# AIGeeksGroup/UniVid

Hardware: AMD Instinct MI355X
Metric: denoise_steps_per_sec (higher is better)
Workload: dtype bf16

## Files before the change

### include/univid_hip.h

```cpp
#ifndef UNIVID_HIP_H
#define UNIVID_HIP_H
#include <stdint.h>
#ifdef __cplusplus
extern "C" {
#endif

int uv_version(void);
const char* uv_build_id(void);
int uv_init(void);
const char* uv_last_error(void);
int uv_device_arch(char* buf, int len);
int uv_host_blocking_sync(int on);

#define UV_OPT_CONV_HALO 0
#define UV_OPT_GEMM_GM 1
#define UV_OPT_ATTN_CUT 2
int uv_set_option(int key, int value);
int uv_get_option(int key, int* value);
int uv_reset_options(void);

#define UV_EPI_BF16 0
#define UV_EPI_GELU_BF16 1
#define UV_EPI_F32_FROM_BF16 2
#define UV_EPI_RESID_F32 3
#define UV_EPI_GATE_RESID_F32 4
#define UV_EPI_BF16_T 5

int uv_gemm_bf16_nt(const void* A, long lda, const void* W, long ldw, const void* bias_bf16, int M, int N, int K,
                    int epilogue, void* out, long ldo, const float* gate, const int32_t* gate_tid, long gate_stride,
                    int tile_cfg, void* stream);

int uv_gemm_bf16_nt_ws(const void* A, long lda, const void* W, long ldw, const void* bias_bf16, int M, int N, int K,
                       int epilogue, void* out, long ldo, const float* gate, const int32_t* gate_tid, long gate_stride,
                       int tile_cfg, void* workspace, long workspace_bytes, void* stream);
long uv_gemm_splitk_ws_bytes(int M, int N, int K);

int uv_gemm_f16_nt(const void* A, long lda, const void* W, long ldw, const void* bias_f16, int M, int N, int K, int epilogue,
                   void* out, long ldo, const float* gate, const int32_t* gate_tid, long gate_stride, int tile_cfg, void* stream);

int uv_gemm_bf16_nt_ssq(const void* A, long lda, const void* W, long ldw, const void* bias_bf16, int M, int N, int K, void* out, long ldo,
                        float* ssq, long ld_ssq, int tile_cfg, void* stream);
int uv_rms_scale_from_ssq(const float* ssq, long ld_ssq, int M, int groups, int C, float eps, float* rs, void* stream);

int uv_gemm_f32_nt(const float* A, long lda, const float* W, long ldw, const float* bias, int M, int N, int K, float* out,
                   long ldo, const float* resid, long ldr, void* stream);

int uv_flash_attn_bf16(const void* q, long ldq, const void* k, long ldk, const void* vt, long ldvt, void* out, long ldo,
                       int batch, int Lq, int Lk, int H, int head_dim, float softmax_scale, void* stream);

int uv_flash_attn_bf16_qnorm(const void* q, long ldq, const void* k, long ldk, const void* vt, long ldvt, void* out, long ldo,
                             int batch, int Lq, int Lk, int H, int head_dim, float softmax_scale, const float* q_rs, const float* q_weight,
                             void* stream);

int uv_flash_attn_f16(const void* q, long ldq, const void* k, long ldk, const void* vt, long ldvt, void* out, long ldo,
                      int batch, int Lq, int Lk, int H, int head_dim, float softmax_scale, void* stream);

int uv_flash_attn_kernel_name(int Lk, int head_dim, long ldk, long ldvt, int f16, char* buf, int len);

int uv_transpose_16(const void* in, long ldi, void* out, long ldo, int L, int C, int Lpad, void* stream);
int uv_cast_f32_to16(const float* in, void* out, long n, int f16, void* stream);
int uv_cast_16_to_f32(const void* in, float* out, long n, int f16, void* stream);

int uv_t5_attention_bf16(const void* q, long ldq, const void* k, long ldk, const void* v, long ldv, void* out, long ldo, int n, int H,
                         const float* rel_bias, int span, void* stream);

int uv_layernorm_mod(const float* x, long ldx, void* out, long ldo, int L, int C, float eps, int mode, const float* tab,
                     long tab_stride, int shift_off, int scale_off, const int32_t* tid, const float* w, const float* b,
                     int round_ln, int out_bf16, void* stream);
// ... 67 lines not shown
```

### univid_amd/_lib.py

```python
import ctypes
import os

import torch

_HERE = os.path.dirname(os.path.abspath(__file__))
LIB_PATH = os.path.join(_HERE, "libunivid_hip.so")

_c = ctypes
_P, _L, _I, _F = _c.c_void_p, _c.c_long, _c.c_int, _c.c_float

SIGNATURES = {
    "uv_version": [],
    "uv_init": [],
    "uv_last_error": [],
    "uv_build_id": [],
    "uv_device_arch": [_c.c_char_p, _I],
    "uv_host_blocking_sync": [_I],
    "uv_set_option": [_I, _I],
    "uv_get_option": [_I, _c.POINTER(_I)],
    "uv_reset_options": [],
    "uv_gemm_bf16_nt": [_P, _L, _P, _L, _P, _I, _I, _I, _I, _P, _L, _P, _P, _L, _I, _P],
    "uv_gemm_bf16_nt_ws": [_P, _L, _P, _L, _P, _I, _I, _I, _I, _P, _L, _P, _P, _L, _I, _P, _L, _P],
    "uv_gemm_splitk_ws_bytes": [_I, _I, _I],
    "uv_gemm_f16_nt": [_P, _L, _P, _L, _P, _I, _I, _I, _I, _P, _L, _P, _P, _L, _I, _P],
    "uv_gemm_f32_nt": [_P, _L, _P, _L, _P, _I, _I, _I, _P, _L, _P, _L, _P],
    "uv_gemm_bf16_nt_ssq": [_P, _L, _P, _L, _P, _I, _I, _I, _P, _L, _P, _L, _I, _P],
    "uv_rms_scale_from_ssq": [_P, _L, _I, _I, _I, _F, _P, _P],
    "uv_flash_attn_bf16_qnorm": [_P, _L, _P, _L, _P, _L, _P, _L, _I, _I, _I, _I, _I, _F, _P, _P, _P],
    "uv_flash_attn_bf16": [_P, _L, _P, _L, _P, _L, _P, _L, _I, _I, _I, _I, _I, _F, _P],
    "uv_flash_attn_f16": [_P, _L, _P, _L, _P, _L, _P, _L, _I, _I, _I, _I, _I, _F, _P],
    "uv_flash_attn_kernel_name": [_I, _I, _L, _L, _I, _c.c_char_p, _I],
    "uv_transpose_16": [_P, _L, _P, _L, _I, _I, _I, _P],
    "uv_cast_f32_to16": [_P, _P, _L, _I, _P],
    "uv_cast_16_to_f32": [_P, _P, _L, _I, _P],
    "uv_layernorm_mod": [_P, _L, _P, _L, _I, _I, _F, _I, _P, _L, _I, _I, _P, _P, _P, _I, _I, _P],
    "uv_t5_attention_bf16": [_P, _L, _P, _L, _P, _L, _P, _L, _I, _I, _P, _I, _P],
    "uv_add_bf16": [_P, _P, _P, _L, _P],
    "uv_t5_gated_gelu_bf16": [_P, _P, _P, _L, _P],
    "uv_gelu_erf_bf16": [_P, _P, _L, _P],
    "uv_interp_linear_rows_bf16": [_P, _L, _P, _L, _I, _I, _I, _P],
    "uv_l2_normalize_rows_f32": [_P, _L, _P, _L, _I, _I, _F, _P],
    "uv_rmsnorm_rope": [_P, _L, _P, _L, _P, _I, _I, _I, _F, _P, _I, _I, _I, _I, _P],
    "uv_rmsnorm_rope_qk": [_P, _P, _P, _P, _P, _P, _L, _L, _I, _I, _I, _I, _F, _P, _I, _I, _I, _I, _P],
    "uv_patchify_bf16": [_P, _P, _L, _I, _I, _I, _I, _I, _I, _I, _I, _P],
    "uv_unpatchify_f32": [_P, _L, _P, _I, _I, _I, _I, _I, _I, _I, _P],
    "uv_sinusoid_f32": [_P, _P, _I, _I, _P],
    "uv_linear_rows_f32": [_P, _L, _P, _P, _P, _L, _I, _I, _I, _I, _P],
    "uv_add_rows_f32": [_P, _P, _P, _I, _L, _P],
    "uv_cast_f32_bf16": [_P, _P, _L, _P],
    "uv_add_bf16_resid": [_P, _L, _P, _L, _I, _I, _P],
    "uv_text_weight_rows_bf16": [_P, _L, _P, _L, _I, _I, _I, _F, _P],
    "uv_cfg_convert": [_P, _P, _P, _F, _F, _P, _P, _L, _P],
    "uv_unipc_corrector": [_P, _P, _P, _P, _P, _F, _F, _F, _F, _F, _F, _I, _L, _P],
    "uv_unipc_predictor": [_P, _P, _P, _P, _F, _F, _F, _F, _I, _L, _P],
    "uv_dpmpp_update": [_P, _P, _P, _P, _F, _F, _F, _I, _L, _P],
    "uv_conv3d_f32": [_P, _L, _I, _I, _I, _P, _P, _P, _L, _I, _I, _I, _I, _I, _I, _I, _I, _I, _I, _I, _I, _I, _I, _I, _I,
# ... 157 lines not shown
        raise UnividHipError(f"{name} failed ({rc}): {lib.uv_last_error().decode()}")
    if timed:
        e.record(stream)
        prof.setdefault(name, []).append((s, e, flops))



def _chk(t, dtype, name):
    if t.device.type != "cuda":
        raise UnividHipError(f"{name}: tensor must live on the GPU (got {t.device})")
    if t.dtype != dtype:
        raise UnividHipError(f"{name}: expected {dtype}, got {t.dtype}")
    if t.stride(-1) != 1:
        raise UnividHipError(f"{name}: innermost dimension must be contiguous")


def host_blocking_sync(on=True, device=None):
    dev = torch.device("cuda" if device is None else device)
    idx = torch.cuda.current_device() if dev.index is None else dev.index
    lib = load()
    with torch.cuda.device(idx):
        if lib.uv_host_blocking_sync(1 if on else 0) != 0:
            raise UnividHipError(lib.uv_last_error().decode())


def gemm_splitk_ws_bytes(M, N, K, device=None):
    dev = torch.device("cuda" if device is None else device)
    idx = torch.cuda.current_device() if dev.index is None else dev.index
    lib = init(idx)
    with torch.cuda.device(idx):
        return int(lib.uv_gemm_splitk_ws_bytes(int(M), int(N), int(K)))


def gemm_bf16(a, w, bias, out, epi, M=None, gate=None, gate_tid=None, tile_cfg=0, ws=None):
    f16 = a.dtype == torch.float16
    _chk(a, torch.float16 if f16 else torch.bfloat16, "gemm_bf16.a")
    _chk(w, a.dtype, "gemm_bf16.w")
    M = a.shape[0] if M is None else M
    N, K = w.shape
    if ws is not None and not f16:
        _chk(ws, torch.uint8, "gemm_bf16.ws")
        call("uv_gemm_bf16_nt_ws", ptr(a), a.stride(0), ptr(w), w.stride(0), ptr(bias), M, N, K, epi, ptr(out), out.stride(0),
             ptr(gate), ptr(gate_tid), 0 if gate is None else gate.stride(0), tile_cfg, ptr(ws), ws.numel(), stream_ptr(), flops=2 * M * N * K)
        return out
    call("uv_gemm_f16_nt" if f16 else "uv_gemm_bf16_nt", ptr(a), a.stride(0), ptr(w), w.stride(0), ptr(bias), M, N, K, epi, ptr(out), out.stride(0),
         ptr(gate), ptr(gate_tid), 0 if gate is None else gate.stride(0), tile_cfg, stream_ptr(), flops=2 * M * N * K)
    return out


def gemm_bf16_ssq(a, w, bias, out, ssq, M=None, tile_cfg=0):
    _chk(a, torch.bfloat16, "gemm_bf16_ssq.a")
    _chk(w, torch.bfloat16, "gemm_bf16_ssq.w")
    _chk(ssq, torch.float32, "gemm_bf16_ssq.ssq")
    M = a.shape[0] if M is None else M
    N, K = w.shape
    call("uv_gemm_bf16_nt_ssq", ptr(a), a.stride(0), ptr(w), w.stride(0), ptr(bias), M, N, K, ptr(out), out.stride(0), ptr(ssq), ssq.stride(0),
         tile_cfg, stream_ptr(), flops=2 * M * N * K)
    return out


def rms_scale_from_ssq(ssq, rs, M, C, eps):
    _chk(ssq, torch.float32, "rms_scale_from_ssq.ssq")
    _chk(rs, torch.float32, "rms_scale_from_ssq.rs")
    call("uv_rms_scale_from_ssq", ptr(ssq), ssq.stride(0), M, ssq.shape[1], C, float(eps), ptr(rs), stream_ptr())
    return rs

# ... 69 lines not shown
```

### univid_amd/csrc/gemm_bf16.hip

```cpp
#include "gemm_bf16_kernels.h"

int uv_gemm_diag_launch(const GemmArgs& a, int epilogue, int tile_cfg, hipStream_t s);

static int num_cus() { return uv_num_cus(); }

template <bool F16>
static int launch_by_cfg(const GemmArgs& a, int epilogue, int tile_cfg, hipStream_t s);

struct GemmWs {
    void* p = nullptr;
    long bytes = 0;
};

template <bool F16>
static bool strip_takes_splitk(const GemmArgs& at, int epilogue, const GemmWs& ws) {
    if (F16 || !ws.p) return false;
    if (epilogue != UV_EPI_BF16 && epilogue != UV_EPI_RESID_F32 && epilogue != UV_EPI_GATE_RESID_F32) return false;
    if (at.K < 8192 || at.K % 512 != 0 || at.N % 256 != 0) return false;
    const long tiles = (long)((at.M + 255) / 256) * (at.N / 256);
    return tiles * 4 <= num_cus() && ws.bytes >= splitk_ws_bytes(at.M, at.N, 4) && ((uintptr_t)ws.p & 255) == 0;
}

static long persistent_rows(int M, int N, bool* short_round) {
    const long tn = N / 256, tm_full = M / 256;
// ... 19 lines not shown
    if (a.gate_tid) at.gate_tid = a.gate_tid + m_main;
    if (epilogue == UV_EPI_BF16_T) at.out = (bf16_t*)a.out + m_main;
    else if (epilogue == UV_EPI_BF16 || epilogue == UV_EPI_GELU_BF16 || epilogue == UV_EPI_BF16_SSQ) at.out = (bf16_t*)a.out + m_main * a.ldo;
    else at.out = (float*)a.out + m_main * a.ldo;
    if (a.ssq) at.ssq = a.ssq + m_main * a.ld_ssq;
    const int rc = launch_by_cfg<F16>(am, epilogue, main_cfg, s);
    if (rc) return rc;
    if constexpr (!F16)
        if (strip_takes_splitk<F16>(at, epilogue, ws)) return launch_8ph_splitk<4, false>(at, epilogue, s, ws.p, ws.bytes);
    return launch_by_cfg<F16>(at, epilogue, 12, s);
}

template <bool F16>
static int gemm_entry(const void* A, long lda, const void* W, long ldw, const void* bias_bf16, int M, int N, int K, int epilogue,
                      void* out, long ldo, const float* gate, const int32_t* gate_tid, long gate_stride, int tile_cfg, void* stream,
                      float* ssq = nullptr, long ld_ssq = 0, const GemmWs& ws = GemmWs()) {
    UV_CHECK_ARG(A && W && out, "uv_gemm_bf16_nt: null pointer");
    UV_CHECK_ARG(M > 0 && N > 0 && K > 0, "uv_gemm_bf16_nt: bad shape M=%d N=%d K=%d", M, N, K);
    UV_CHECK_ARG(K % UV_BK == 0, "uv_gemm_bf16_nt: K=%d must be a multiple of %d", K, UV_BK);
    UV_CHECK_ARG(N % 16 == 0, "uv_gemm_bf16_nt: N=%d must be a multiple of 16", N);
    UV_CHECK_ARG(lda % 8 == 0 && ldw % 8 == 0, "uv_gemm_bf16_nt: lda/ldw must be multiples of 8 elements");
    UV_CHECK_ARG(((uintptr_t)A & 15) == 0 && ((uintptr_t)W & 15) == 0 && ((uintptr_t)out & 15) == 0,
                 "uv_gemm_bf16_nt: pointers must be 16-byte aligned");
    UV_CHECK_ARG(ldo % 4 == 0, "uv_gemm_bf16_nt: ldo must be a multiple of 4 elements");
    if (epilogue == UV_EPI_GATE_RESID_F32)
        UV_CHECK_ARG(gate && gate_stride % 4 == 0, "uv_gemm_bf16_nt: gate table required (stride %% 4 == 0)");
    GemmArgs a;
    a.A = (const bf16_t*)A; a.W = (const bf16_t*)W; a.bias = (const bf16_t*)bias_bf16;
    a.out = out; a.gate = gate; a.gate_tid = gate_tid;
    a.lda = lda; a.ldw = ldw; a.ldo = ldo; a.gate_stride = gate_stride;
    a.M = M; a.N = N; a.K = K; a.tiles_m = a.tiles_n = 0;
    a.ssq = ssq; a.ld_ssq = ld_ssq;
    a.ws_slab = nullptr; a.ws_cnt = nullptr; a.gm = 0;
    if (epilogue == UV_EPI_BF16_SSQ)
        UV_CHECK_ARG(ssq && N % 32 == 0 && ld_ssq >= N / 32 && ldo % 8 == 0, "uv_gemm_bf16_nt_ssq: needs N %% 32 == 0, ld_ssq >= N / 32, ldo %% 8 == 0 (N=%d ld_ssq=%ld ldo=%ld)", N, ld_ssq, ldo);
    a.zeros = uv_zero_page();
    UV_CHECK_ARG(a.zeros, "uv_gemm_bf16_nt: zero page missing (call uv_init)");
    hipStream_t s = (hipStream_t)stream;
    if (tile_cfg == 0 && M >= 2048 && N >= 1024 && N % 256 == 0 && K % 128 == 0 && K >= 384 &&
        (ldo % 8 == 0 || epilogue == UV_EPI_BF16_T || (epilogue >= UV_EPI_F32_FROM_BF16 && epilogue != UV_EPI_BF16_SSQ))) {
        const long tn = N / 256;
        bool short_round = false;
        const long m_main = persistent_rows(M, N, &short_round);
        if (m_main / 256 * tn < 2L * num_cus() || (epilogue == UV_EPI_BF16_T && ldo % 8 != 0)) {
            if (short_round) return launch_m_split<F16>(a, epilogue, 7, s);
            return launch_by_cfg<F16>(a, epilogue, 7, s);
        }
        return launch_m_split<F16>(a, epilogue, 17, s, m_main, ws);
    }
    if constexpr (!F16) {
        if (tile_cfg == 19) return launch_8ph_splitk<4, false>(a, epilogue, s, ws.p, ws.bytes);
        if (tile_cfg == 20) return launch_8ph_splitk<2, false>(a, epilogue, s, ws.p, ws.bytes);
        if (tile_cfg == 21) { a.gm = 1; return launch_8ph_splitk<4, false>(a, epilogue, s, ws.p, ws.bytes); }
    }
    if (tile_cfg == 8) return launch_m_split<F16>(a, epilogue, 7, s);
    if (tile_cfg == 9) return launch_m_split<F16>(a, epilogue, 5, s);
    if (tile_cfg == 18) return launch_m_split<F16>(a, epilogue, 17, s, (long)(M / 256) * 256 < M ? (long)(M / 256) * 256 : 0);
    return launch_by_cfg<F16>(a, epilogue, tile_cfg, s);
}

extern "C" int uv_gemm_bf16_nt(const void* A, long lda, const void* W, long ldw, const void* bias_bf16,
                               int M, int N, int K, int epilogue, void* out, long ldo,
                               const float* gate, const int32_t* gate_tid, long gate_stride,
                               int tile_cfg, void* stream) {
    return gemm_entry<false>(A, lda, W, ldw, bias_bf16, M, N, K, epilogue, out, ldo, gate, gate_tid, gate_stride, tile_cfg, stream);
}

extern "C" int uv_gemm_bf16_nt_ws(const void* A, long lda, const void* W, long ldw, const void* bias_bf16,
                                  int M, int N, int K, int epilogue, void* out, long ldo,
                                  const float* gate, const int32_t* gate_tid, long gate_stride,
                                  int tile_cfg, void* workspace, long workspace_bytes, void* stream) {
    UV_CHECK_ARG(workspace_bytes >= 0 && (workspace || workspace_bytes == 0), "uv_gemm_bf16_nt_ws: bad workspace");
    GemmWs ws;
    ws.p = workspace; ws.bytes = workspace_bytes;
    return gemm_entry<false>(A, lda, W, ldw, bias_bf16, M, N, K, epilogue, out, ldo, gate, gate_tid, gate_stride, tile_cfg, stream, nullptr, 0, ws);
}

extern "C" long uv_gemm_splitk_ws_bytes(int M, int N, int K) {
    if (M < 2048 || N < 1024 || N % 256 != 0 || K < 8192 || K % 512 != 0) return 0;
    const long tn = N / 256;
    bool short_round = false;
    const long m_main = persistent_rows(M, N, &short_round);
    if (m_main / 256 * tn < 2L * num_cus() || m_main >= M) return 0;
    const long strip_tiles = ((M - m_main) + 255) / 256 * tn;
    return strip_tiles * 4 <= num_cus() ? splitk_ws_bytes((int)(M - m_main), N, 4) : 0;
}

extern "C" int uv_gemm_bf16_nt_ssq(const void* A, long lda, const void* W, long ldw, const void* bias_bf16, int M, int N, int K,
                                   void* out, long ldo, float* ssq, long ld_ssq, int tile_cfg, void* stream) {
    return gemm_entry<false>(A, lda, W, ldw, bias_bf16, M, N, K, UV_EPI_BF16_SSQ, out, ldo, nullptr, nullptr, 0, tile_cfg, stream, ssq, ld_ssq);
}

extern "C" int uv_gemm_f16_nt(const void* A, long lda, const void* W, long ldw, const void* bias_f16,
                              int M, int N, int K, int epilogue, void* out, long ldo,
                              const float* gate, const int32_t* gate_tid, long gate_stride,
                              int tile_cfg, void* stream) {
    UV_CHECK_ARG(tile_cfg == 0, "uv_gemm_f16_nt: only tile_cfg 0 (automatic) is built for fp16 operands");
    return gemm_entry<true>(A, lda, W, ldw, bias_f16, M, N, K, epilogue, out, ldo, gate, gate_tid, gate_stride, tile_cfg, stream);
}

template <bool F16>
static int launch_by_cfg(const GemmArgs& a, int epilogue, int tile_cfg, hipStream_t s) {
    const int M = a.M, N = a.N, K = a.K;
    switch (tile_cfg) {
        case 0: {
            if (M < 2048 || N < 1024) {
                if (M >= 4096 && N >= 512 && N % 256 == 0 && K % 128 == 0 && K >= 256 && a.ldo % 8 == 0 && a.M % 256 == 0 &&
                    2L * (M / 256) * (N / 256) >= num_cus())
                    return launch_8ph<5, F16>(a, epilogue, s);
                const long t128 = (long)((M + 127) / 128) * ((N + 127) / 128);
                if (t128 <= 2 * num_cus()) return launch_cfg<128, 128, 4, 2, 4, F16>(a, epilogue, s);
                return launch_cfg<128, 128, 2, 2, 2, F16>(a, epilogue, s);
            }
            const long tm = (M + 255) / 256;
            const long t256 = tm * ((N + 255) / 256), t192 = tm * ((N + 191) / 192);
            const double c256 = (double)((t256 + 255) / 256) * 1.00, c192 = (double)((t192 + 255) / 256) * 0.78;
            if (!F16 && N % 192 == 0 && c192 < c256 && K <= 4096 && epilogue != UV_EPI_BF16_SSQ) return launch_cfg<256, 192, 4, 4>(a, epilogue, s);
            return launch_cfg<256, 256, 4, 4, 2, F16>(a, epilogue, s);
        }
        case 1: if constexpr (!F16) return launch_cfg<128, 128, 2, 2>(a, epilogue, s); else break;
        case 5: if constexpr (!F16) return launch_cfg<256, 256, 4, 4>(a, epilogue, s); else break;
        case 6: if constexpr (!F16) return launch_cfg<256, 192, 4, 4>(a, epilogue, s); else break;
        case 12: return launch_cfg<128, 128, 4, 2, 4, F16>(a, epilogue, s);
        case 7:
            UV_CHECK_ARG(K % 128 == 0 && K >= 256, "uv_gemm_bf16_nt: tile_cfg 7 needs K %% 128 == 0 and K >= 256 (K=%d)", K);
            return launch_8ph<5, F16>(a, epilogue, s);
        case 17:
            UV_CHECK_ARG(K % 128 == 0 && K >= 384, "uv_gemm_bf16_nt: tile_cfg 17 needs K %% 128 == 0 and K >= 384 (K=%d)", K);
            return launch_8ph_persist<F16>(a, epilogue, s);
        default:
            if constexpr (!F16) return uv_gemm_diag_launch(a, epilogue, tile_cfg, s);
            else break;
    }
    uv_set_error("uv_gemm_f16_nt: tile_cfg %d is not built for fp16 operands", tile_cfg);
    return -1;
}
```

### univid_amd/csrc/gemm_bf16_kernels.h

```cpp
#pragma once
#include "common.h"
#include <stdlib.h>

const float* uv_zero_page();

#define UV_BK 64

enum {
    UV_EPI_BF16 = 0,
    UV_EPI_GELU_BF16 = 1,
    UV_EPI_F32_FROM_BF16 = 2,
    UV_EPI_RESID_F32 = 3,
    UV_EPI_GATE_RESID_F32 = 4,
    UV_EPI_BF16_T = 5,
    UV_EPI_BF16_SSQ = 6,
};

struct GemmArgs {
    const bf16_t* A;
    const bf16_t* W;
    const bf16_t* bias;
    void* out;
    const float* gate;
    const int32_t* gate_tid;
    const float* zeros;
    long lda, ldw, ldo, gate_stride;
    int M, N, K;
    int tiles_m, tiles_n;
    int gm;
    float* ssq;
    long ld_ssq;
    float* ws_slab;
    int* ws_cnt;
};

typedef __attribute__((address_space(3))) void lds_void;

__device__ __forceinline__ void glds16(const void* g, lds_void* l) {
    __builtin_amdgcn_global_load_lds(g, l, 16, 0, 0);
}

template <int EPI, bool F16 = false, bool FULL = false>
__device__ __forceinline__ void epi_frag(const GemmArgs& p, int mb, int nb, const f32x4& a, int frow, int fq) {
    if (EPI != UV_EPI_BF16_T) {
        const int m = mb + frow, n = nb + 4 * fq;
        if (!FULL && (m >= p.M || n >= p.N)) return;
        float v[4];
#pragma unroll
        for (int e = 0; e < 4; ++e) v[e] = a[e];
        if (FULL || p.bias) {
            const u32x2 bb = *(const u32x2*)((FULL && !p.bias) ? (const bf16_t*)p.zeros : p.bias + n);
            v[0] += in16<F16>((bf16_t)(bb[0] & 0xffff));
            v[1] += in16<F16>((bf16_t)(bb[0] >> 16));
            v[2] += in16<F16>((bf16_t)(bb[1] & 0xffff));
            v[3] += in16<F16>((bf16_t)(bb[1] >> 16));
        }
        if (EPI == UV_EPI_BF16) {
            u32x2 o = {pack16_2<F16>(v[0], v[1]), pack16_2<F16>(v[2], v[3])};
            *(u32x2*)((bf16_t*)p.out + (long)m * p.ldo + n) = o;
        } else if (EPI == UV_EPI_GELU_BF16) {
#pragma unroll
            for (int e = 0; e < 4; e += 2) {
                const uint32_t pk = pack16_2<F16>(v[e], v[e + 1]);
                const f32x2 y = gelu_tanh_f32x2((f32x2){in16<F16>((bf16_t)(pk & 0xffff)), in16<F16>((bf16_t)(pk >> 16))});
                v[e] = y[0];
                v[e + 1] = y[1];
// ... 129 lines not shown
        for (int f = 0; f < NF; ++f) t[f] = p.gate_tid ? p.gate_tid[min(mb[f] + frow, p.M - 1)] : 0;
#pragma unroll
        for (int f = 0; f < NF; ++f) grow[f] = p.gate + (long)t[f] * p.gate_stride;
    }
    f32x4 xb[D], gb[D];
    u32x2 bb[D];
    auto issue = [&](int f, int slot) {
        const int m = min(mb[f] + frow, p.M - 1), n = min(nb[f] + 4 * fq, p.N - 4);
        xb[slot] = *(const f32x4*)((const float*)p.out + (long)m * p.ldo + n);
        if (GATE) gb[slot] = *(const f32x4*)(grow[f] + n);
        bb[slot] = p.bias ? *(const u32x2*)(p.bias + n) : (u32x2){0u, 0u};
    };
#pragma unroll
    for (int f = 0; f < D && f < NF; ++f) issue(f, f);
#pragma unroll
    for (int f = 0; f < NF; ++f) {
        const int slot = f % D;
        const int m = mb[f] + frow, n = nb[f] + 4 * fq;
        float v[4];
        v[0] = acc[f][0] + in16<F16>((bf16_t)(bb[slot][0] & 0xffff));
        v[1] = acc[f][1] + in16<F16>((bf16_t)(bb[slot][0] >> 16));
        v[2] = acc[f][2] + in16<F16>((bf16_t)(bb[slot][1] & 0xffff));
        v[3] = acc[f][3] + in16<F16>((bf16_t)(bb[slot][1] >> 16));
        f32x4 x = xb[slot];
#pragma unroll
        for (int e = 0; e < 4; ++e)
            x[e] = GATE ? __fadd_rn(x[e], __fmul_rn(round16<F16>(v[e]), gb[slot][e])) : __fadd_rn(x[e], round16<F16>(v[e]));
        if (m < p.M && n < p.N) *(f32x4*)((float*)p.out + (long)m * p.ldo + n) = x;
        if (f + D < NF) issue(f + D, slot);
    }
}

template <int BM, int BN, int WM, int WN, int EPI, int NS = 2, bool F16 = false>
__global__ __launch_bounds__(WM* WN * 64) void gemm_bf16_nt_kernel(GemmArgs p) {
    constexpr int NW = WM * WN;
    constexpr int NT = NW * 64;
    constexpr int TM = BM / WM / 16;
    constexpr int TN = BN / WN / 16;
    constexpr int A_BYTES = BM * 128;
    constexpr int W_BYTES = BN * 128;
    constexpr int STAGE_BYTES = A_BYTES + W_BYTES;
    constexpr int A_INSTR = (BM / 8 + NW - 1) / NW;
    constexpr int W_INSTR = (BN / 8 + NW - 1) / NW;
    static_assert(BM % 8 == 0 && BN % 8 == 0 && (BM / WM) % 16 == 0 && (BN / WN) % 16 == 0, "tile/wave mismatch");
    constexpr bool TRANS = (EPI == UV_EPI_BF16_T);

    extern __shared__ __attribute__((aligned(16))) char smem[];

    const int tid = threadIdx.x;
    const int lane = tid & 63;
    const int wave = __builtin_amdgcn_readfirstlane(tid >> 6);
    const int wm = wave / WN, wn = wave % WN;

    const int nblk = p.tiles_m * p.tiles_n;
    int bid = blockIdx.x;
    {
        const int q = nblk >> 3, r = nblk & 7, xcd = bid & 7, idx = bid >> 3;
        bid = (xcd < r ? xcd * (q + 1) : r * (q + 1) + (xcd - r) * q) + idx;
    }
    constexpr int GM = 4;
    const int group_sz = GM * p.tiles_n;
    const int group = bid / group_sz;
    const int first_m = group * GM;
    const int gm = min(GM, p.tiles_m - first_m);
    const int in_group = bid - group * group_sz;
    const int tile_m = first_m + in_group % gm;
    const int tile_n = in_group / gm;
    const int m0 = tile_m * BM, n0 = tile_n * BN;

    const int srow = lane >> 3;
    const int pchunk = lane & 7;
    const bf16_t* a_src[A_INSTR];
    const bf16_t* w_src[W_INSTR];
#pragma unroll
    for (int i = 0; i < A_INSTR; ++i) {
        const int row = (i * NW + wave) * 8 + srow;
        const int c = pchunk ^ ((row >> 1) & 7);
        const int gr = min(m0 + row, p.M - 1);
        a_src[i] = p.A + (long)gr * p.lda + c * 8;
    }
#pragma unroll
    for (int i = 0; i < W_INSTR; ++i) {
        const int row = (i * NW + wave) * 8 + srow;
        const int c = pchunk ^ ((row >> 1) & 7);
        const int gr = min(n0 + row, p.N - 1);
        w_src[i] = p.W + (long)gr * p.ldw + c * 8;
    }

    auto stage = [&](int kt, int buf) {
        char* base = smem + buf * STAGE_BYTES;
        const int koff = kt * UV_BK;
#pragma unroll
        for (int i = 0; i < A_INSTR; ++i)
            if ((i * NW + wave) * 8 < BM) glds16(a_src[i] + koff, (lds_void*)(base + (i * NW + wave) * 1024));
#pragma unroll
        for (int i = 0; i < W_INSTR; ++i)
            if ((i * NW + wave) * 8 < BN) glds16(w_src[i] + koff, (lds_void*)(base + A_BYTES + (i * NW + wave) * 1024));
    };

    f32x4 acc[TN][TM];
#pragma unroll
// ... 71 lines not shown
            compute(smem + buf * STAGE_BYTES);
            buf = buf + 1 == NS ? 0 : buf + 1;
            nbuf = nbuf + 1 == NS ? 0 : nbuf + 1;
        }
    }

    if constexpr (EPI == UV_EPI_RESID_F32 || EPI == UV_EPI_GATE_RESID_F32) {
        constexpr int NF = TM * TN;
        int mb[NF], nb[NF];
        f32x4 av[NF];
#pragma unroll
        for (int j = 0; j < TM; ++j)
#pragma unroll
            for (int i = 0; i < TN; ++i) {
                mb[j * TN + i] = m0 + wm * (BM / WM) + j * 16;
                nb[j * TN + i] = n0 + wn * (BN / WN) + i * 16;
                av[j * TN + i] = acc[i][j];
            }
        epi_rmw_pipe<EPI, NF, (NF >= 8 ? 4 : 2), F16>(p, mb, nb, av, frow, fq);
    } else if constexpr (EPI == UV_EPI_BF16_SSQ) {
        static_assert(TN % 2 == 0 && (BN / WN) % 32 == 0, "UV_EPI_BF16_SSQ needs whole 32-column groups per wave");
#pragma unroll
        for (int j = 0; j < TM; ++j)
#pragma unroll
            for (int i = 0; i < TN; i += 2)
                epi_pair_ssq<F16>(p, m0 + wm * (BM / WM) + j * 16, n0 + wn * (BN / WN) + i * 16, acc[i][j], acc[i + 1][j], frow, fq);
    } else {
#pragma unroll
        for (int j = 0; j < TM; ++j)
#pragma unroll
            for (int i = 0; i < TN; ++i)
                epi_frag<EPI, F16>(p, m0 + wm * (BM / WM) + j * 16, n0 + wn * (BN / WN) + i * 16, acc[i][j], frow, fq);
    }
}


template <int EPI, bool F16>
__device__ __forceinline__ void epi_rmw_rows_lds(const GemmArgs& p, char* smem, const f32x4 (&acc)[2][2][2][4], int m0, int n0,
                                                 int wave, int lane) {
    static_assert(EPI == UV_EPI_RESID_F32 || EPI == UV_EPI_GATE_RESID_F32, "rmw epilogues only");
    constexpr bool GATE = EPI == UV_EPI_GATE_RESID_F32;
    constexpr int D = 8;
    const int wr = wave >> 2, wc = wave & 3;
    const int frow = lane & 15, fq = lane >> 4;
    float bv[2][2][4];
#pragma unroll
    for (int hn = 0; hn < 2; ++hn)
#pragma unroll
        for (int i = 0; i < 2; ++i) {
            const int n = min(n0 + hn * 128 + wc * 32 + i * 16 + 4 * fq, p.N - 4);
            const u32x2 bb = p.bias ? *(const u32x2*)(p.bias + n) : (u32x2){0u, 0u};
            bv[hn][i][0] = in16<F16>((bf16_t)(bb[0] & 0xffff));
            bv[hn][i][1] = in16<F16>((bf16_t)(bb[0] >> 16));
            bv[hn][i][2] = in16<F16>((bf16_t)(bb[1] & 0xffff));
            bv[hn][i][3] = in16<F16>((bf16_t)(bb[1] >> 16));
        }
    const int n = n0 + 4 * lane;
    const bool n_ok = n < p.N;
    const int nc = min(n, p.N - 4);
#pragma unroll
    for (int h = 0; h < 2; ++h) {
#pragma unroll
        for (int j = 0; j < 4; ++j)
#pragma unroll
            for (int hn = 0; hn < 2; ++hn)
#pragma unroll
// ... 313 lines not shown
#pragma unroll
            for (int j = 0; j < 4; ++j)
#pragma unroll
                for (int hn = 0; hn < 2; ++hn)
#pragma unroll
                    for (int i = 0; i < 2; ++i)
                        epi_frag<EPI, F16>(p, m0 + hm * 128 + wr * 64 + j * 16, n0 + hn * 128 + wc * 32 + i * 16, acc[hn][hm][i][j], frow, fq);
    }
}

template <int EPI, bool F16 = false>
__global__ __launch_bounds__(512) void gemm_bf16_8ph_persist_kernel(GemmArgs p) {
    constexpr bool TRANS = (EPI == UV_EPI_BF16_T);
    constexpr bool RMW = (EPI == UV_EPI_RESID_F32 || EPI == UV_EPI_GATE_RESID_F32);
    constexpr int VAR = 5;
    constexpr int HALF = 16384;
    constexpr int BUF = 4 * HALF;
    extern __shared__ __attribute__((aligned(16))) char smem[];

    const int tid = threadIdx.x;
    const int lane = tid & 63;
    const int wave = __builtin_amdgcn_readfirstlane(tid >> 6);
    const int wr = wave >> 2, wc = wave & 3;

    const int nblk = p.tiles_m * p.tiles_n;
    const int G = gridDim.x >> 3;
    int first, cnt;
    {
        const int q = nblk >> 3, r = nblk & 7, xcd = blockIdx.x & 7;
        first = xcd < r ? xcd * (q + 1) : r * (q + 1) + (xcd - r) * q;
        cnt = q + (xcd < r ? 1 : 0);
    }
    int cur = blockIdx.x >> 3;
    if (cur >= cnt) return;
    const int GM = p.gm;
    const int group_sz = GM * p.tiles_n;
    auto origin = [&](int bid, int& m0, int& n0) {
        const int group = bid / group_sz;
        const int first_m = group * GM;
        const int gm = min(GM, p.tiles_m - first_m);
        const int in_group = bid - group * group_sz;
        m0 = (first_m + in_group % gm) * 256;
        n0 = (in_group / gm) * 256;
    };
    int m0, n0;
    origin(first + cur, m0, n0);

    const int srow = lane >> 3, pchunk = lane & 7;
    const bf16_t* a_src[2][2];
    const bf16_t* w_src[2][2];
#pragma unroll
    for (int h = 0; h < 2; ++h)
#pragma unroll
        for (int i = 0; i < 2; ++i) {
            const int row = (i * 8 + wave) * 8 + srow;
            const int c = pchunk ^ ((row >> 1) & 7);
            a_src[h][i] = p.A + (long)(m0 + h * 128 + row) * p.lda + c * 8;
            w_src[h][i] = p.W + (long)(n0 + h * 128 + row) * p.ldw + c * 8;
        }
    char* const my_dst = smem + wave * 1024;
    const int nk = p.K / UV_BK;
    const int frow = lane & 15, fq = lane >> 4;
    const int lx = (fq ^ (frow >> 1)) << 4;
    const char* const la = smem + (wr * 64 + frow) * 128;
    const char* const lw = smem + 2 * HALF + (wc * 32 + frow) * 128;
    f32x4 acc[2][2][2][4];
    bf16x8 af[4][2], w0[2][2], w1[2][2];

    auto move_ptrs = [&](const bf16_t* (&src)[2], long d) { src[0] += d; src[1] += d; };
    bool fresh = true;
    for (;;) {
        if (fresh) {
            UV_STAGE(w_src[0], 0, 2 * HALF) UV_STAGE(w_src[1], 0, 3 * HALF) UV_STAGE(a_src[0], 0, 0) UV_STAGE(a_src[1], 0, HALF)
            if (!UV_REBAL) UV_STAGE(w_src[0], 1, BUF + 2 * HALF)
            UV_STAGE(w_src[1], 1, BUF + 3 * HALF) UV_STAGE(a_src[0], 1, BUF)
            if (UV_REBAL) asm volatile("s_waitcnt vmcnt(6)" ::: "memory");
            else asm volatile("s_waitcnt vmcnt(8)" ::: "memory");
            UV_SB();
        }
        fresh = RMW;
        if (wr == 1) UV_SB();
#pragma unroll
        for (int a = 0; a < 2; ++a)
#pragma unroll
            for (int b = 0; b < 2; ++b)
#pragma unroll
                for (int i = 0; i < 2; ++i)
#pragma unroll
                    for (int j = 0; j < 4; ++j) acc[a][b][i][j] = (f32x4){0.f, 0.f, 0.f, 0.f};

        const int nxt = cur + G;
        const bool has_next = nxt < cnt;
        int m1 = m0, n1 = n0;
        long dA = 0, dW = 0;
        if (has_next) {
            origin(first + nxt, m1, n1);
            dA = (long)(m1 - m0) * p.lda;
            dW = (long)(n1 - n0) * p.ldw;
        }
        int t = 0;
        for (; t + 2 < nk; t += 2) {
            UV_KTILE5(t, 0, 1, true, true)
            UV_KTILE5(t + 1, 1, 0, true, true)
        }
// ... 20 lines not shown
                __builtin_amdgcn_s_barrier();
            }
        } else if constexpr (EPI == UV_EPI_BF16 || EPI == UV_EPI_GELU_BF16 || EPI == UV_EPI_BF16_SSQ) {
#pragma unroll
            for (int hm = 0; hm < 2; ++hm)
#pragma unroll
                for (int j = 0; j < 4; ++j)
#pragma unroll
                    for (int hn = 0; hn < 2; ++hn)
                        epi_pair16<EPI, F16>(p, m0 + hm * 128 + wr * 64 + j * 16, n0 + hn * 128 + wc * 32, acc[hn][hm][0][j], acc[hn][hm][1][j], frow, fq);
        } else if constexpr (EPI == UV_EPI_BF16_T) {
#pragma unroll
            for (int hm = 0; hm < 2; ++hm)
#pragma unroll
                for (int j = 0; j < 4; j += 2)
#pragma unroll
                    for (int hn = 0; hn < 2; ++hn)
#pragma unroll
                        for (int i = 0; i < 2; ++i)
                            epi_pair16_T<F16>(p, m0 + hm * 128 + wr * 64 + j * 16, n0 + hn * 128 + wc * 32 + i * 16, acc[hn][hm][i][j], acc[hn][hm][i][j + 1], frow, fq);
        } else {
#pragma unroll
            for (int hm = 0; hm < 2; ++hm)
#pragma unroll
                for (int j = 0; j < 4; ++j)
#pragma unroll
                    for (int hn = 0; hn < 2; ++hn)
#pragma unroll
                        for (int i = 0; i < 2; ++i)
                            epi_frag<EPI, F16, true>(p, m0 + hm * 128 + wr * 64 + j * 16, n0 + hn * 128 + wc * 32 + i * 16, acc[hn][hm][i][j], frow, fq);
        }
        if (!has_next) break;
        m0 = m1; n0 = n1; cur = nxt;
    }
    asm volatile("s_waitcnt vmcnt(0)" ::: "memory");
}

template <int VAR = 0, bool F16 = false>
static int launch_8ph(const GemmArgs& a0, int epi, hipStream_t stream) {
    GemmArgs a = a0;
    a.tiles_m = (a.M + 255) / 256;
    a.tiles_n = (a.N + 255) / 256;
    const dim3 grid(a.tiles_m * a.tiles_n), block(512);
    const size_t lds = 128 * 1024;
#define UV_LAUNCH8(E)                                                                              \
    case E: {                                                                                      \
        auto kern = gemm_bf16_8ph_kernel<E, VAR, F16>;                                               \
        UV_ONCE_PER_DEVICE(hipFuncSetAttribute((const void*)kern, hipFuncAttributeMaxDynamicSharedMemorySize, (int)lds));  \
        hipLaunchKernelGGL(kern, grid, block, lds, stream, a);                                     \
        break;                                                                                     \
    }
    switch (epi) {
        UV_LAUNCH8(UV_EPI_BF16)
        UV_LAUNCH8(UV_EPI_GELU_BF16)
        UV_LAUNCH8(UV_EPI_F32_FROM_BF16)
        UV_LAUNCH8(UV_EPI_RESID_F32)
        UV_LAUNCH8(UV_EPI_GATE_RESID_F32)
        UV_LAUNCH8(UV_EPI_BF16_T)
        UV_LAUNCH8(UV_EPI_BF16_SSQ)
        default:
            uv_set_error("uv_gemm_bf16_nt: unknown epilogue %d", epi);
            return -1;
    }
#undef UV_LAUNCH8
    UV_CHECK_LAUNCH("uv_gemm_bf16_nt");
    return 0;
// ... 11 lines not shown
    UV_CHECK_ARG(tiles <= 1024, "uv_gemm_bf16_nt_ws: split-K serves leftover strips (at most 1024 tiles; %d here)", tiles);
    UV_CHECK_ARG(ws && ((uintptr_t)ws & 255) == 0 && ws_bytes >= splitk_ws_bytes(a.M, a.N, SK),
                 "uv_gemm_bf16_nt_ws: workspace of %ld bytes (256-byte aligned) needed, %ld given", splitk_ws_bytes(a.M, a.N, SK), ws_bytes);
    a.ws_cnt = (int*)ws;
    a.ws_slab = (float*)((char*)ws + 4096);
    if (hipMemsetAsync(a.ws_cnt, 0, (size_t)tiles * sizeof(int), stream) != hipSuccess) {
        uv_set_error("uv_gemm_bf16_nt_ws: hipMemsetAsync of the tile counters failed");
        return -1;
    }
    const int per = a.gm == 0 ? (tiles * SK + 7) / 8 : (tiles + 8 / SK - 1) / (8 / SK);
    const dim3 grid(8 * per), block(512);
    const size_t lds = 128 * 1024;
#define UV_LAUNCH8S(E)                                                                             \
    case E: {                                                                                      \
        auto kern = gemm_bf16_8ph_kernel<E, 5, F16, SK>;                                           \
        UV_ONCE_PER_DEVICE(hipFuncSetAttribute((const void*)kern, hipFuncAttributeMaxDynamicSharedMemorySize, (int)lds));  \
        hipLaunchKernelGGL(kern, grid, block, lds, stream, a);                                     \
        break;                                                                                     \
    }
    switch (epi) {
        UV_LAUNCH8S(UV_EPI_BF16)
        UV_LAUNCH8S(UV_EPI_RESID_F32)
        UV_LAUNCH8S(UV_EPI_GATE_RESID_F32)
        default:
            uv_set_error("uv_gemm_bf16_nt_ws: the split-K strip is built for the bf16 and the residual epilogues (0, 3, 4), not %d", epi);
            return -1;
    }
#undef UV_LAUNCH8S
    UV_CHECK_LAUNCH("uv_gemm_bf16_nt_ws");
    return 0;
}

template <bool F16 = false>
static int launch_8ph_persist(const GemmArgs& a0, int epi, hipStream_t stream) {
    GemmArgs a = a0;
    UV_CHECK_ARG(a.M % 256 == 0 && a.N % 256 == 0, "uv_gemm_bf16_nt: the persistent kernel needs whole 256x256 tiles (M=%d N=%d)", a.M, a.N);
    UV_CHECK_ARG(a.ldo % 8 == 0 || (epi != UV_EPI_BF16_T && epi != UV_EPI_BF16 && epi != UV_EPI_GELU_BF16 && epi != UV_EPI_BF16_SSQ),
                 "uv_gemm_bf16_nt: the persistent kernel stores 16 bytes per lane: ldo=%ld must be a multiple of 8 elements", a.ldo);
    a.tiles_m = a.M / 256;
    a.tiles_n = a.N / 256;
    a.gm = (a.N <= 4096 && a.K <= 4096) ? 8 : (a.K >= 8192 ? 2 : 4);
    if (const int gm = uv_option(UV_OPT_GEMM_GM); gm > 0) a.gm = gm;
    const int tiles = a.tiles_m * a.tiles_n;
    int wgs = uv_num_cus() & ~7;
    if (wgs > tiles) wgs = tiles & ~7;
    UV_CHECK_ARG(wgs >= 8, "uv_gemm_bf16_nt: too few tiles (%d) for the persistent kernel", tiles);
    const dim3 grid(wgs), block(512);
    const size_t lds = 128 * 1024;
#define UV_LAUNCH8P(E)                                                                             \
    case E: {                                                                                      \
        auto kern = gemm_bf16_8ph_persist_kernel<E, F16>;                                          \
        UV_ONCE_PER_DEVICE(hipFuncSetAttribute((const void*)kern, hipFuncAttributeMaxDynamicSharedMemorySize, (int)lds));  \
        hipLaunchKernelGGL(kern, grid, block, lds, stream, a);                                     \
        break;                                                                                     \
    }
    switch (epi) {
        UV_LAUNCH8P(UV_EPI_BF16)
        UV_LAUNCH8P(UV_EPI_GELU_BF16)
        UV_LAUNCH8P(UV_EPI_F32_FROM_BF16)
        UV_LAUNCH8P(UV_EPI_RESID_F32)
        UV_LAUNCH8P(UV_EPI_GATE_RESID_F32)
        UV_LAUNCH8P(UV_EPI_BF16_T)
        UV_LAUNCH8P(UV_EPI_BF16_SSQ)
        default:
            uv_set_error("uv_gemm_bf16_nt: unknown epilogue %d", epi);
            return -1;
    }
#undef UV_LAUNCH8P
    UV_CHECK_LAUNCH("uv_gemm_bf16_nt");
    return 0;
}

template <int BM, int BN, int WM, int WN, int NS = 2, bool F16 = false>
// ... 40 lines not shown
```

Baseline: 3.997.

## Fold GEMM row-tail tiles into the persistent kernel instead of a second launch

Instead of splitting M into a persistent main part and a separately launched strip, the persistent 256x256 kernel now also processes the leftover rows as 128x128 tail tiles. Workgroups that received fewer main tiles take the first tail units, and the rest are spread round-robin. This removes a second kernel launch and the idle tail of the main round. Split-K is still used when the strip qualifies, and tile_cfg 22 forces the old path. A launch-count query is added for callers.

New measurement: 4.007 (median of 6 runs). About the same (+0.2%).

```diff
diff --git a/include/univid_hip.h b/include/univid_hip.h
--- a/include/univid_hip.h
+++ b/include/univid_hip.h
@@ -34,6 +34,7 @@
                        int epilogue, void* out, long ldo, const float* gate, const int32_t* gate_tid, long gate_stride,
                        int tile_cfg, void* workspace, long workspace_bytes, void* stream);
 long uv_gemm_splitk_ws_bytes(int M, int N, int K);
+int uv_gemm_launch_count(int M, int N, int K, int epilogue);
 
 int uv_gemm_f16_nt(const void* A, long lda, const void* W, long ldw, const void* bias_f16, int M, int N, int K, int epilogue,
                    void* out, long ldo, const float* gate, const int32_t* gate_tid, long gate_stride, int tile_cfg, void* stream);
diff --git a/univid_amd/_lib.py b/univid_amd/_lib.py
--- a/univid_amd/_lib.py
+++ b/univid_amd/_lib.py
@@ -22,6 +22,7 @@
     "uv_gemm_bf16_nt": [_P, _L, _P, _L, _P, _I, _I, _I, _I, _P, _L, _P, _P, _L, _I, _P],
     "uv_gemm_bf16_nt_ws": [_P, _L, _P, _L, _P, _I, _I, _I, _I, _P, _L, _P, _P, _L, _I, _P, _L, _P],
     "uv_gemm_splitk_ws_bytes": [_I, _I, _I],
+    "uv_gemm_launch_count": [_I, _I, _I, _I],
     "uv_gemm_f16_nt": [_P, _L, _P, _L, _P, _I, _I, _I, _I, _P, _L, _P, _P, _L, _I, _P],
     "uv_gemm_f32_nt": [_P, _L, _P, _L, _P, _I, _I, _I, _P, _L, _P, _L, _P],
     "uv_gemm_bf16_nt_ssq": [_P, _L, _P, _L, _P, _I, _I, _I, _P, _L, _P, _L, _I, _P],
@@ -245,6 +246,14 @@
         return int(lib.uv_gemm_splitk_ws_bytes(int(M), int(N), int(K)))
 
 
+def gemm_launch_count(M, N, K, epi, device=None):
+    dev = torch.device("cuda" if device is None else device)
+    idx = torch.cuda.current_device() if dev.index is None else dev.index
+    lib = init(idx)
+    with torch.cuda.device(idx):
+        return int(lib.uv_gemm_launch_count(int(M), int(N), int(K), int(epi)))
+
+
 def gemm_bf16(a, w, bias, out, epi, M=None, gate=None, gate_tid=None, tile_cfg=0, ws=None):
     f16 = a.dtype == torch.float16
     _chk(a, torch.float16 if f16 else torch.bfloat16, "gemm_bf16.a")
diff --git a/univid_amd/csrc/gemm_bf16.hip b/univid_amd/csrc/gemm_bf16.hip
--- a/univid_amd/csrc/gemm_bf16.hip
+++ b/univid_amd/csrc/gemm_bf16.hip
@@ -75,12 +75,13 @@
     a.M = M; a.N = N; a.K = K; a.tiles_m = a.tiles_n = 0;
     a.ssq = ssq; a.ld_ssq = ld_ssq;
     a.ws_slab = nullptr; a.ws_cnt = nullptr; a.gm = 0;
+    a.tail_m0 = a.tail_units = a.tail_first = 0;
     if (epilogue == UV_EPI_BF16_SSQ)
         UV_CHECK_ARG(ssq && N % 32 == 0 && ld_ssq >= N / 32 && ldo % 8 == 0, "uv_gemm_bf16_nt_ssq: needs N %% 32 == 0, ld_ssq >= N / 32, ldo %% 8 == 0 (N=%d ld_ssq=%ld ldo=%ld)", N, ld_ssq, ldo);
     a.zeros = uv_zero_page();
     UV_CHECK_ARG(a.zeros, "uv_gemm_bf16_nt: zero page missing (call uv_init)");
     hipStream_t s = (hipStream_t)stream;
-    if (tile_cfg == 0 && M >= 2048 && N >= 1024 && N % 256 == 0 && K % 128 == 0 && K >= 384 &&
+    if ((tile_cfg == 0 || tile_cfg == 22) && M >= 2048 && N >= 1024 && N % 256 == 0 && K % 128 == 0 && K >= 384 &&
         (ldo % 8 == 0 || epilogue == UV_EPI_BF16_T || (epilogue >= UV_EPI_F32_FROM_BF16 && epilogue != UV_EPI_BF16_SSQ))) {
         const long tn = N / 256;
         bool short_round = false;
@@ -89,7 +90,10 @@
             if (short_round) return launch_m_split<F16>(a, epilogue, 7, s);
             return launch_by_cfg<F16>(a, epilogue, 7, s);
         }
-        return launch_m_split<F16>(a, epilogue, 17, s, m_main, ws);
+        GemmArgs at = a;
+        at.M = M - (int)m_main;
+        if (tile_cfg == 22 || (m_main < M && strip_takes_splitk<F16>(at, epilogue, ws))) return launch_m_split<F16>(a, epilogue, 17, s, m_main, ws);
+        return launch_8ph_persist<F16>(a, epilogue, s, m_main);
     }
     if constexpr (!F16) {
         if (tile_cfg == 19) return launch_8ph_splitk<4, false>(a, epilogue, s, ws.p, ws.bytes);
@@ -127,6 +131,21 @@
     if (m_main / 256 * tn < 2L * num_cus() || m_main >= M) return 0;
     const long strip_tiles = ((M - m_main) + 255) / 256 * tn;
     return strip_tiles * 4 <= num_cus() ? splitk_ws_bytes((int)(M - m_main), N, 4) : 0;
+}
+
+extern "C" int uv_gemm_launch_count(int M, int N, int K, int epilogue) {
+    if (!(M >= 2048 && N >= 1024 && N % 256 == 0 && K % 128 == 0 && K >= 384)) return 1;
+    const long tn = N / 256;
+    bool short_round = false;
+    const long m_main = persistent_rows(M, N, &short_round);
+    if (m_main / 256 * tn < 2L * num_cus()) {
+        if (!short_round) return 1;
+        const long rounds = (long)((M + 255) / 256) * tn / num_cus();
+        const long cut = rounds * num_cus() / tn * 256;
+        return rounds > 0 && cut > 0 && cut < M ? 2 : 1;
+    }
+    (void)epilogue;
+    return 1;
 }
 
 extern "C" int uv_gemm_bf16_nt_ssq(const void* A, long lda, const void* W, long ldw, const void* bias_bf16, int M, int N, int K,
@@ -170,7 +189,7 @@
             return launch_8ph<5, F16>(a, epilogue, s);
         case 17:
             UV_CHECK_ARG(K % 128 == 0 && K >= 384, "uv_gemm_bf16_nt: tile_cfg 17 needs K %% 128 == 0 and K >= 384 (K=%d)", K);
-            return launch_8ph_persist<F16>(a, epilogue, s);
+            return launch_8ph_persist<F16>(a, epilogue, s, M / 256 * 256);
         default:
             if constexpr (!F16) return uv_gemm_diag_launch(a, epilogue, tile_cfg, s);
             else break;
diff --git a/univid_amd/csrc/gemm_bf16_kernels.h b/univid_amd/csrc/gemm_bf16_kernels.h
--- a/univid_amd/csrc/gemm_bf16_kernels.h
+++ b/univid_amd/csrc/gemm_bf16_kernels.h
@@ -32,6 +32,9 @@
     long ld_ssq;
     float* ws_slab;
     int* ws_cnt;
+    int tail_m0;
+    int tail_units;
+    int tail_first;
 };
 
 typedef __attribute__((address_space(3))) void lds_void;
@@ -227,7 +230,7 @@
 }
 
 template <int BM, int BN, int WM, int WN, int EPI, int NS = 2, bool F16 = false>
-__global__ __launch_bounds__(WM* WN * 64) void gemm_bf16_nt_kernel(GemmArgs p) {
+__device__ __forceinline__ void nt_tile(const GemmArgs& p, char* smem, int m0, int n0) {
     constexpr int NW = WM * WN;
     constexpr int NT = NW * 64;
     constexpr int TM = BM / WM / 16;
@@ -240,28 +243,10 @@
     static_assert(BM % 8 == 0 && BN % 8 == 0 && (BM / WM) % 16 == 0 && (BN / WN) % 16 == 0, "tile/wave mismatch");
     constexpr bool TRANS = (EPI == UV_EPI_BF16_T);
 
-    extern __shared__ __attribute__((aligned(16))) char smem[];
-
     const int tid = threadIdx.x;
     const int lane = tid & 63;
     const int wave = __builtin_amdgcn_readfirstlane(tid >> 6);
     const int wm = wave / WN, wn = wave % WN;
-
-    const int nblk = p.tiles_m * p.tiles_n;
-    int bid = blockIdx.x;
-    {
-        const int q = nblk >> 3, r = nblk & 7, xcd = bid & 7, idx = bid >> 3;
-        bid = (xcd < r ? xcd * (q + 1) : r * (q + 1) + (xcd - r) * q) + idx;
-    }
-    constexpr int GM = 4;
-    const int group_sz = GM * p.tiles_n;
-    const int group = bid / group_sz;
-    const int first_m = group * GM;
-    const int gm = min(GM, p.tiles_m - first_m);
-    const int in_group = bid - group * group_sz;
-    const int tile_m = first_m + in_group % gm;
-    const int tile_n = in_group / gm;
-    const int m0 = tile_m * BM, n0 = tile_n * BN;
 
     const int srow = lane >> 3;
     const int pchunk = lane & 7;
@@ -399,6 +384,26 @@
             for (int i = 0; i < TN; ++i)
                 epi_frag<EPI, F16>(p, m0 + wm * (BM / WM) + j * 16, n0 + wn * (BN / WN) + i * 16, acc[i][j], frow, fq);
     }
+}
+
+template <int BM, int BN, int WM, int WN, int EPI, int NS = 2, bool F16 = false>
+__global__ __launch_bounds__(WM* WN * 64) void gemm_bf16_nt_kernel(GemmArgs p) {
+    extern __shared__ __attribute__((aligned(16))) char smem[];
+    const int nblk = p.tiles_m * p.tiles_n;
+    int bid = blockIdx.x;
+    {
+        const int q = nblk >> 3, r = nblk & 7, xcd = bid & 7, idx = bid >> 3;
+        bid = (xcd < r ? xcd * (q + 1) : r * (q + 1) + (xcd - r) * q) + idx;
+    }
+    constexpr int GM = 4;
+    const int group_sz = GM * p.tiles_n;
+    const int group = bid / group_sz;
+    const int first_m = group * GM;
+    const int gm = min(GM, p.tiles_m - first_m);
+    const int in_group = bid - group * group_sz;
+    const int tile_m = first_m + in_group % gm;
+    const int tile_n = in_group / gm;
+    nt_tile<BM, BN, WM, WN, EPI, NS, F16>(p, smem, tile_m * BM, tile_n * BN);
 }
 
 
@@ -778,7 +783,6 @@
         cnt = q + (xcd < r ? 1 : 0);
     }
     int cur = blockIdx.x >> 3;
-    if (cur >= cnt) return;
     const int GM = p.gm;
     const int group_sz = GM * p.tiles_n;
     auto origin = [&](int bid, int& m0, int& n0) {
@@ -815,7 +819,7 @@
 
     auto move_ptrs = [&](const bf16_t* (&src)[2], long d) { src[0] += d; src[1] += d; };
     bool fresh = true;
-    for (;;) {
+    if (cur < cnt) for (;;) {
         if (fresh) {
             UV_STAGE(w_src[0], 0, 2 * HALF) UV_STAGE(w_src[1], 0, 3 * HALF) UV_STAGE(a_src[0], 0, 0) UV_STAGE(a_src[1], 0, HALF)
             if (!UV_REBAL) UV_STAGE(w_src[0], 1, BUF + 2 * HALF)
@@ -902,6 +906,34 @@
         }
         if (!has_next) break;
         m0 = m1; n0 = n1; cur = nxt;
+    }
+
+    if (p.tail_units > 0) {
+        const int q = nblk >> 3, r = nblk & 7, xcd = blockIdx.x & 7, cur0 = blockIdx.x >> 3;
+        const int L = (q + (r ? 1 : 0) + G - 1) / G;
+        int heavy = 0, heavy_before = 0, light_before = 0, my_heavy = 0;
+        for (int x = 0; x < 8; ++x) {
+            const int h = min(max(q + (x < r ? 1 : 0) - (L - 1) * G, 0), G);
+            if (x < xcd) { heavy_before += h; light_before += G - h; }
+            if (x == xcd) my_heavy = h;
+            heavy += h;
+        }
+        const int W = gridDim.x, T = p.tail_units;
+        const int nlight = W - heavy;
+        const bool is_heavy = cur0 < my_heavy;
+        const int lrank = light_before + cur0 - my_heavy;
+        const int t1 = min(nlight * p.tail_first, T);
+        const int u_lo = is_heavy ? 0 : min(lrank * p.tail_first, t1);
+        const int n1 = is_heavy ? 0 : min(u_lo + p.tail_first, t1) - u_lo;
+        const int order = is_heavy ? heavy_before + cur0 : heavy + lrank;
+        const int tm_t = (p.M - p.tail_m0 + 127) / 128;
+        for (int k = 0;; ++k) {
+            const int u = k < n1 ? u_lo + k : t1 + order + (k - n1) * W;
+            if (u >= T) break;
+            asm volatile("s_waitcnt vmcnt(0) lgkmcnt(0)" ::: "memory");
+            __builtin_amdgcn_s_barrier();
+            nt_tile<128, 128, 4, 2, EPI, 4, F16>(p, smem, p.tail_m0 + (u % tm_t) * 128, (u / tm_t) * 128);
+        }
     }
     asm volatile("s_waitcnt vmcnt(0)" ::: "memory");
 }
@@ -979,13 +1011,17 @@
 }
 
 template <bool F16 = false>
-static int launch_8ph_persist(const GemmArgs& a0, int epi, hipStream_t stream) {
+static int launch_8ph_persist(const GemmArgs& a0, int epi, hipStream_t stream, long m_main = 0) {
     GemmArgs a = a0;
-    UV_CHECK_ARG(a.M % 256 == 0 && a.N % 256 == 0, "uv_gemm_bf16_nt: the persistent kernel needs whole 256x256 tiles (M=%d N=%d)", a.M, a.N);
+    if (m_main <= 0) m_main = a.M;
+    UV_CHECK_ARG(m_main % 256 == 0 && m_main <= a.M && a.N % 256 == 0, "uv_gemm_bf16_nt: the persistent kernel needs whole 256x256 tiles (M=%d rows %ld N=%d)", a.M, m_main, a.N);
     UV_CHECK_ARG(a.ldo % 8 == 0 || (epi != UV_EPI_BF16_T && epi != UV_EPI_BF16 && epi != UV_EPI_GELU_BF16 && epi != UV_EPI_BF16_SSQ),
                  "uv_gemm_bf16_nt: the persistent kernel stores 16 bytes per lane: ldo=%ld must be a multiple of 8 elements", a.ldo);
-    a.tiles_m = a.M / 256;
+    a.tiles_m = (int)(m_main / 256);
     a.tiles_n = a.N / 256;
+    a.tail_m0 = (int)m_main;
+    a.tail_units = (int)((a.M - m_main + 127) / 128) * (a.N / 128);
+    a.tail_first = 3;
     a.gm = (a.N <= 4096 && a.K <= 4096) ? 8 : (a.K >= 8192 ? 2 : 4);
     if (const int gm = uv_option(UV_OPT_GEMM_GM); gm > 0) a.gm = gm;
     const int tiles = a.tiles_m * a.tiles_n;
```
